# Andreas-Edling/raytracer-rs

Measured on AMD Instinct MI355X. Metric: Mrays/s (whole node) + ms/frame, 1920x1080x64spp thai2.dae, higher is better.
Workload: dtype f32

## Files before the change

### raytracer-rs_amd/csrc/kernels.hip

```cpp
#include <hip/hip_runtime.h>
#include <algorithm>
#include <stdint.h>
#include <stdlib.h>
#include <map>
#include <mutex>
#include <utility>
#include "device_math.hpp"
#include "device_types.hpp"
#include "kernels.hpp"
#include "lens.hpp"
#include "reflmask.hpp"
#include "traverse.hpp"

namespace mi355rt {

typedef const uint32_t __attribute__((address_space(4))) * const_u1_ptr;
constexpr int kBlock = 256;
constexpr int kWavesPerBlock = kBlock / 64;
constexpr uint32_t kMiss = 0xFFFFFFFFu;
constexpr int kPrimaryBlocks = 7;
#ifndef MI355RT_WIDE_BLOCKS
#define MI355RT_WIDE_BLOCKS 5
#endif
constexpr int kConfirmBlocks = 5;
// ... 842 lines not shown
                        float4 tv0 = table[jx0], tv1 = table[jx1];
                        hemisphere_walk(table, n, jx0, tv0);
                        if (two) hemisphere_walk(table, n, jx1, tv1);
                        bd0 = mk3(tv0.x, tv0.y, tv0.z); bo0 = add3(hp, sscale(0.00001f, bd0));
                        bd1 = mk3(tv1.x, tv1.y, tv1.z); bo1 = add3(hp, sscale(0.00001f, bd1));
                    }
                    bool make0 = active, make1 = active && two;
                    if (sc.refl_mask != nullptr) {
                        if (make0) make0 = !reflection_proves_miss(sc, refl_rec, n, bo0, bd0);
                        if (make1) make1 = !reflection_proves_miss(sc, refl_rec, n, bo1, bd1);
                        bskipped += (uint32_t)__popcll(__ballot(active && !make0)) + (uint32_t)__popcll(__ballot(active && two && !make1));
                    }
                    uint32_t pos[2] = { 0u, 0u };
                    const uint32_t key0 = make0 ? dir_bin(bd0) : kSortBins, key1 = make1 ? dir_bin(bd1) : kSortBins;
                    for (uint32_t b = 0; b < kSortBins; ++b) {
                        const unsigned long long m0 = __ballot(key0 == b), m1 = __ballot(key1 == b);
                        if (key0 == b) pos[0] = out_front + (uint32_t)__popcll(m0 & lanemask_lt());
                        out_front += (uint32_t)__popcll(m0);
                        if (key1 == b) pos[1] = out_front + (uint32_t)__popcll(m1 & lanemask_lt());
                        out_front += (uint32_t)__popcll(m1);
                    }
                    for (uint32_t w = 0; w < (two ? 2u : 1u); ++w) {
                        const f3 bo = w ? bo1 : bo0, bd = w ? bd1 : bd0;
                        const uint32_t child_node = w ? child1 : child0;
                        const uint32_t oi = pos[w];
                        if ((w ? make1 : make0) && oi + out_back < ps.region + 0u) {
                            const size_t r = base + oi;
                            st4<2>(&out_q[r], make_float4(bo.x, bo.y, bo.z, bd.x));
                            st4<2>(&out_q[ps.qstride + r], make_float4(bd.y, bd.z, __uint_as_float(slot), __uint_as_float(((level + 1u) << 4) | (child_node << 8))));
                        }
                    }
                }
            }
        }
        __builtin_amdgcn_wave_barrier();
        if (out_front + out_back > ps.region) { if (lane == 0) counters->overflow = 1u; out_front = 0u; out_back = 0u; }
        if (out_counts != nullptr && lane == 0) out_counts[chunk] = make_uint2(out_front, out_back);
        out_nrad = out_front; out_nshadow = out_back;
        acc_bounce += out_front + ((unsigned long long)bskipped << 32); acc_shadow += out_back + ((unsigned long long)skipped << 32); acc_hits += cnt - dropped;
    }
}

__device__ __forceinline__ void flush_shade_counters(DCounters* counters, uint32_t wave, unsigned long long acc_bounce, unsigned long long acc_shadow, unsigned long long acc_hits)
{
    if (lane_id() == 0) {
        DCounters* cs = &counters[wave % kShards];
        if (acc_bounce & 0xFFFFFFFFull) atomicAdd(&cs->bounce, acc_bounce & 0xFFFFFFFFull);
        if (acc_bounce >> 32) atomicAdd(&cs->bounce_skipped, acc_bounce >> 32);
        if (acc_shadow & 0xFFFFFFFFull) atomicAdd(&cs->shadow, acc_shadow & 0xFFFFFFFFull);
        if (acc_shadow >> 32) atomicAdd(&cs->shadow_skipped, acc_shadow >> 32);
        if (acc_hits & 0xFFFFFFFFull) atomicAdd(&cs->primary_hits, acc_hits & 0xFFFFFFFFull);
        if (acc_hits >> 32) atomicAdd(&cs->primary_culled, acc_hits >> 32);
    }
}

template <bool PRIMARY, bool WALK, bool RASTER = false, uint32_t RAYS = kFeedCamera>
__global__ __launch_bounds__(kBlock, PRIMARY ? (WALK ? kShadePWBlocks : kShadePBlocks) : (WALK ? kShadeSWBlocks : kShadeSBlocks)) void shade_kernel(DScene sc, DCamera cam, DPass ps, uint32_t level,
                                                      const float4* __restrict__ in_q, const uint2* __restrict__ in_counts,
                                                      const float4* __restrict__ hits,
                                                      float4* __restrict__ out_q, uint2* __restrict__ out_counts, uint32_t* cursor,
                                                      float* __restrict__ slot_L, uint32_t* __restrict__ sample_slot,
                                                      const uint32_t* __restrict__ film_n, DCounters* counters)
{
    extern __shared__ uint32_t s_list[];
    const LinearList list{ &s_list[(threadIdx.x >> 6) * ps.list_cap] };
    float4* lds_hits = RASTER ? (float4*)&s_list[kWavesPerBlock * ps.list_cap] + (threadIdx.x >> 6) * ps.chunk : nullptr;
    const uint32_t wave = blockIdx.x * kWavesPerBlock + (threadIdx.x >> 6);
    unsigned long long acc_bounce = 0, acc_shadow = 0, acc_hits = 0, acc_tris = 0;
    PullState pull; uint32_t chunk = 0u;
    while (pull_chunk(cursor, ps.nchunks, pull, chunk, 0u, PRIMARY ? LiveLists() : live_lists(ps))) {
        uint32_t o_rad, o_sh;
        shade_chunk<PRIMARY, LinearList, WALK, RASTER, RAYS>(sc, cam, ps, level, chunk, list, in_q, PRIMARY ? 0u : in_counts[chunk].x, o_rad, o_sh, hits, out_q, out_counts, slot_L, sample_slot, film_n, counters, acc_bounce, acc_shadow, acc_hits,
                                                       lds_hits, (RASTER && (ps.flags & 2u)) ? &acc_tris : nullptr);
        if (PRIMARY && ps.live != nullptr && (o_rad | o_sh) != 0u && lane_id() == 0) {
            const uint32_t k = chunk % kMaxCursors;
            const uint32_t at = atomicAdd(&ps.live_count[(size_t)k * kCursorStride + kLiveCountOffset], 1u);
            ps.live[(size_t)k * ps.live_cap + at] = chunk;
        }
    }
    flush_shade_counters(counters, wave, acc_bounce, acc_shadow, PRIMARY ? acc_hits : 0ull);
    if (RASTER && acc_tris && lane_id() == 0) atomicAdd(&counters[wave % kShards].tris_tested, acc_tris);
}

template <int REC>
__device__ f3 node_radiance(const float* __restrict__ L, const DPass& ps, uint32_t nlights, uint32_t level, uint32_t index)
{
    const uint32_t node = ps.level_first[level] + index;
    f3 rad = mk3(0.0f, 0.0f, 0.0f);
    for (uint32_t li = 0; li < nlights; ++li) {
        const float* p = L + 3ull * ((size_t)node * nlights + li) * ps.nslots;
        rad = add3(rad, mk3(p[0], p[1], p[2]));
    }
    if constexpr (REC == 0) {
        return rad;
    } else {
        const uint32_t k = ps.spread * (uint32_t)REC;
        f3 sum = mk3(0.0f, 0.0f, 0.0f);
        for (uint32_t c = 0; c < k; ++c) sum = add3(sum, node_radiance<REC - 1>(L, ps, nlights, level + 1, index * k + c));
        const f3 sub = vscale(sum, div_rn(1.0f, (float)k));
        return add3(rad, sub);
    }
}

template <uint32_t kResolveLanes, bool DIRECT>
__global__ __launch_bounds__(256) void resolve_kernel(DPass ps, uint32_t width, uint32_t nlights, const float* __restrict__ slot_L,
                                                     const uint32_t* __restrict__ sample_slot,
                                                     float* film_sum, float* film_sumsq, uint32_t* film_n, float* debug_color, uint32_t* ctrl, float* film_direct)
{
    if (ctrl != nullptr && blockIdx.x == 0)
        for (uint32_t i = threadIdx.x; i < kMaxRounds * kMaxCursors * 4u; i += blockDim.x)
            ctrl[(size_t)(i / (kMaxCursors * 4u)) * kCtrlWordsPerRound + (size_t)((i / 4u) % kMaxCursors) * kCursorStride + (i % 4u) * kConfirmCursorOffset] = 0u;
    const uint32_t gid = blockIdx.x * blockDim.x + threadIdx.x;
    const uint32_t j = gid % kResolveLanes;
    const bool live = gid / kResolveLanes < ps.npix;
    const uint32_t p = live ? gid / kResolveLanes : ps.npix - 1u;
    const uint32_t spp = ps.nsamples / ps.npix;
    const uint32_t pixel = ps.use_explicit ? ps.explicit_pixel : pass_pixel(ps, width, p);
    f3 sum = mk3(0, 0, 0), sumsq = mk3(0, 0, 0), direct = mk3(0, 0, 0);
    uint32_t n = 0;
    if (!ps.use_explicit) {
        sum = mk3(film_sum[3ull * pixel], film_sum[3ull * pixel + 1], film_sum[3ull * pixel + 2]);
        sumsq = mk3(film_sumsq[3ull * pixel], film_sumsq[3ull * pixel + 1], film_sumsq[3ull * pixel + 2]);
        n = film_n[pixel];
        if constexpr (DIRECT) direct = mk3(film_direct[3ull * pixel], film_direct[3ull * pixel + 1], film_direct[3ull * pixel + 2]);
    }
    const int group_lane0 = lane_id() & ~(int)(kResolveLanes - 1u);
    const bool dead = ps.block_culled != nullptr && ps.block_culled[(uint32_t)(sample_index(ps, 0u, p) / ps.chunk) % ps.cull_blocks] != 0u;
    const bool on = ps.use_explicit || pixel_active(ps, width, pixel);
    for (uint32_t s0 = 0; s0 < spp; s0 += kResolveLanes) {
        const uint32_t sl = (s0 + j < spp && !dead && on) ? sample_slot[sample_index(ps, s0 + j, p)] : 0xFFFFFFFFu;
        const float* L = slot_L + 3ull * (size_t)sl;
        f3 c = mk3(0.0f, 0.0f, 0.0f);
        if (sl != 0xFFFFFFFFu) switch (ps.recursions) {
            case 0: c = node_radiance<0>(L, ps, nlights, 0, 0); break;
            case 1: c = node_radiance<1>(L, ps, nlights, 0, 0); break;
            case 2: c = node_radiance<2>(L, ps, nlights, 0, 0); break;
            default: c = node_radiance<3>(L, ps, nlights, 0, 0); break;
        }
        f3 d = mk3(0.0f, 0.0f, 0.0f);
        if constexpr (DIRECT) { if (sl != 0xFFFFFFFFu) d = node_radiance<0>(L, ps, nlights, 0, 0); }
#pragma unroll
        for (uint32_t k = 0; k < kResolveLanes; ++k) {
            const f3 ck = mk3(__shfl(c.x, group_lane0 + (int)k, 64), __shfl(c.y, group_lane0 + (int)k, 64), __shfl(c.z, group_lane0 + (int)k, 64));
            f3 dk = mk3(0.0f, 0.0f, 0.0f);
            if constexpr (DIRECT) dk = mk3(__shfl(d.x, group_lane0 + (int)k, 64), __shfl(d.y, group_lane0 + (int)k, 64), __shfl(d.z, group_lane0 + (int)k, 64));
            if (s0 + k < spp) {
                sum = add3(sum, ck);
                sumsq = add3(sumsq, mk3(ck.x * ck.x, ck.y * ck.y, ck.z * ck.z));
                n += 1u;
                if constexpr (DIRECT) direct = add3(direct, dk);
                if (ps.use_explicit && j == 0u) { debug_color[0] = ck.x; debug_color[1] = ck.y; debug_color[2] = ck.z; }
            }
        }
    }
    if (!ps.use_explicit && live && on && j == 0u) {
        film_sum[3ull * pixel] = sum.x; film_sum[3ull * pixel + 1] = sum.y; film_sum[3ull * pixel + 2] = sum.z;
        film_sumsq[3ull * pixel] = sumsq.x; film_sumsq[3ull * pixel + 1] = sumsq.y; film_sumsq[3ull * pixel + 2] = sumsq.z;
        film_n[pixel] = n;
        if constexpr (DIRECT) { film_direct[3ull * pixel] = direct.x; film_direct[3ull * pixel + 1] = direct.y; film_direct[3ull * pixel + 2] = direct.z; }
    }
}

__global__ __launch_bounds__(256) void resolve_rays_kernel(DPass ps, uint32_t nlights, const float* __restrict__ slot_L, const uint32_t* __restrict__ sample_slot,
                                                          float* __restrict__ rgb, float* __restrict__ direct, float* __restrict__ tuv, uint32_t* __restrict__ prim, uint32_t* ctrl)
{
    if (ctrl != nullptr && blockIdx.x == 0)
        for (uint32_t i = threadIdx.x; i < kMaxRounds * kMaxCursors * 4u; i += blockDim.x)
            ctrl[(size_t)(i / (kMaxCursors * 4u)) * kCtrlWordsPerRound + (size_t)((i / 4u) % kMaxCursors) * kCursorStride + (i % 4u) * kConfirmCursorOffset] = 0u;
    const uint32_t i = blockIdx.x * blockDim.x + threadIdx.x;
    if (i >= ps.nsamples) return;
    if (rgb != nullptr || direct != nullptr) {
        const uint32_t sl = sample_slot[i];
        const float* L = slot_L + 3ull * (size_t)sl;
        f3 c = mk3(0.0f, 0.0f, 0.0f), d = mk3(0.0f, 0.0f, 0.0f);
        if (sl != 0xFFFFFFFFu) {
            if (rgb != nullptr) switch (ps.recursions) {
                case 0: c = node_radiance<0>(L, ps, nlights, 0, 0); break;
                case 1: c = node_radiance<1>(L, ps, nlights, 0, 0); break;
                case 2: c = node_radiance<2>(L, ps, nlights, 0, 0); break;
                default: c = node_radiance<3>(L, ps, nlights, 0, 0); break;
            }
            if (direct != nullptr) d = node_radiance<0>(L, ps, nlights, 0, 0);
        }
        if (rgb != nullptr) { rgb[3ull * i] = c.x; rgb[3ull * i + 1] = c.y; rgb[3ull * i + 2] = c.z; }
        if (direct != nullptr) { direct[3ull * i] = d.x; direct[3ull * i + 1] = d.y; direct[3ull * i + 2] = d.z; }
    }
    if (ps.ray_hit != nullptr) {
        const float4 h = ps.ray_hit[i];
        const uint32_t p = __float_as_uint(h.w);
        if (prim != nullptr) prim[i] = p;
        if (tuv != nullptr && p != kMiss) { tuv[3ull * i] = h.x; tuv[3ull * i + 1] = h.y; tuv[3ull * i + 2] = h.z; }
    }
}
hipError_t launch_resolve_rays(hipStream_t stream, const DPass& ps, uint32_t nlights, const float* slot_L, const uint32_t* sample_slot,
                               float* rgb, float* direct, float* tuv, uint32_t* prim, uint32_t* ctrl)
{
    hipLaunchKernelGGL(resolve_rays_kernel, dim3((ps.nsamples + 255u) / 256u ? (ps.nsamples + 255u) / 256u : 1u), dim3(256), 0, stream, ps, nlights, slot_L, sample_slot, rgb, direct, tuv, prim, ctrl);
    return hipGetLastError();
}

__device__ __forceinline__ void phase_fence() { __builtin_amdgcn_fence(__ATOMIC_SEQ_CST, "workgroup"); }

template <bool DIRECT>
__device__ __forceinline__ void resolve_chunk_1spp(const DPass& ps, uint32_t width, uint32_t nlights, uint32_t chunk, const float* slot_L, const uint32_t* sample_slot,
                                                   float* film_sum, float* film_sumsq, uint32_t* film_n, float* film_direct)
{
    const uint32_t n = min(ps.chunk, ps.nsamples - chunk * ps.chunk);
    for (uint32_t i = (uint32_t)lane_id(); i < n; i += 64u) {
        const uint32_t p = chunk * ps.chunk + i;
        const uint32_t pixel = pass_pixel(ps, width, p);
        const uint32_t sl = sample_slot[p];
        const float* L = slot_L + 3ull * (size_t)sl;
        f3 c = mk3(0.0f, 0.0f, 0.0f);
        if (sl != 0xFFFFFFFFu) switch (ps.recursions) {
            case 0: c = node_radiance<0>(L, ps, nlights, 0, 0); break;
            case 1: c = node_radiance<1>(L, ps, nlights, 0, 0); break;
            case 2: c = node_radiance<2>(L, ps, nlights, 0, 0); break;
            default: c = node_radiance<3>(L, ps, nlights, 0, 0); break;
        }
        float* ps_ = film_sum + 3ull * pixel; float* pq = film_sumsq + 3ull * pixel;
        ps_[0] = ps_[0] + c.x; ps_[1] = ps_[1] + c.y; ps_[2] = ps_[2] + c.z;
        pq[0] = pq[0] + c.x * c.x; pq[1] = pq[1] + c.y * c.y; pq[2] = pq[2] + c.z * c.z;
        film_n[pixel] = film_n[pixel] + 1u;
        if constexpr (DIRECT) {
            f3 d = mk3(0.0f, 0.0f, 0.0f);
            if (sl != 0xFFFFFFFFu) d = node_radiance<0>(L, ps, nlights, 0, 0);
            float* pd = film_direct + 3ull * pixel;
            pd[0] = pd[0] + d.x; pd[1] = pd[1] + d.y; pd[2] = pd[2] + d.z;
        }
    }
}

constexpr int kFusedBlocks = 1;
template <bool CONFIRM, bool DIRECT>
__global__ __launch_bounds__(kBlock, kFusedBlocks) void fused_pass_kernel(DScene sc, DCamera cam, DPass ps, float4* q0, float4* q1,
                                                            float4* hits, float* slot_L, uint32_t* sample_slot,
                                                            float* film_sum, float* film_sumsq, uint32_t* film_n, float* film_direct, DCounters* counters)
{
    extern __shared__ int s_stack[];
    int* stack = &s_stack[threadIdx.x];
    const ColumnList list{ &s_stack[threadIdx.x & ~63u] };
    const uint32_t wave = global_wave_id(), nwaves = gridDim.x * kWavesPerBlock;
    unsigned long long acc_bounce = 0, acc_shadow = 0, acc_hits = 0;
    for (uint32_t chunk = wave; chunk < ps.nchunks; chunk += nwaves) {
        uint32_t n_rad = 0u, n_sh = 0u;
        trace_wave<true, false, true, true>(sc, cam, ps, nullptr, nullptr, hits, nullptr, slot_L, film_n, counters, stack, chunk, 0u, 0u);
        phase_fence();
        if (CONFIRM && !sc.oct_single_leaf) { confirm_chunk<true>(sc, cam, ps, chunk, list, nullptr, 0u, 0u, hits, slot_L, film_n); phase_fence(); }
        shade_chunk<true>(sc, cam, ps, 0u, chunk, list, nullptr, 0u, n_rad, n_sh, hits, q0, nullptr, slot_L, sample_slot, film_n, counters, acc_bounce, acc_shadow, acc_hits);
        phase_fence();
        for (uint32_t r = 1; r < ps.recursions + 2u; ++r) {
            float4* in_q = (r - 1u) & 1u ? q1 : q0;
            trace_wave<false, false, true, CONFIRM>(sc, cam, ps, in_q, nullptr, hits, nullptr, slot_L, film_n, counters, stack, chunk, n_rad, n_sh);
            phase_fence();
            if (CONFIRM && !sc.oct_single_leaf) { confirm_chunk<false>(sc, cam, ps, chunk, list, in_q, n_rad, n_sh, hits, slot_L, film_n); phase_fence(); }
            if (r <= ps.recursions) {
                unsigned long long unused = 0;
                uint32_t o_rad = 0u, o_sh = 0u;
                shade_chunk<false>(sc, cam, ps, r, chunk, list, in_q, n_rad, o_rad, o_sh, hits, r & 1u ? q1 : q0, nullptr, slot_L, sample_slot, film_n, counters, acc_bounce, acc_shadow, unused);
                n_rad = o_rad; n_sh = o_sh;
                phase_fence();
            }
        }
        resolve_chunk_1spp<DIRECT>(ps, cam.width, sc.nlights, chunk, slot_L, sample_slot, film_sum, film_sumsq, film_n, film_direct);
    }
    flush_shade_counters(counters, wave, acc_bounce, acc_shadow, acc_hits);
}

__device__ __forceinline__ uint32_t to_u8(float c)
{
    const float m = fmaxf(fminf(c, 1.0f), 0.0f) * 255.0f;
    return (uint32_t)m & 0xFFu;
}
__global__ __launch_bounds__(256) void tonemap_kernel(const uint32_t* __restrict__ rows, uint32_t row_base, uint32_t nrows, uint32_t width, int packed,
                                                     const float* __restrict__ film_sum, const uint32_t* __restrict__ film_n, uint32_t* out)
{
    const size_t i = (size_t)blockIdx.x * blockDim.x + threadIdx.x;
    if (i >= (size_t)nrows * width) return;
    const uint32_t r = (uint32_t)(i / width), x = (uint32_t)(i % width);
    const size_t pixel = (size_t)(rows ? rows[r] : row_base + r) * width + x;
    const float inv = div_rn(1.0f, (float)film_n[pixel]);
    const float cr = film_sum[3 * pixel] * inv, cg = film_sum[3 * pixel + 1] * inv, cb = film_sum[3 * pixel + 2] * inv;
    const uint32_t R = to_u8(div_rn(cr, 1.0f + cr)), G = to_u8(div_rn(cg, 1.0f + cg)), B = to_u8(div_rn(cb, 1.0f + cb));
    out[packed ? i : pixel] = B | (G << 8) | (R << 16) | (255u << 24);
}

__device__ __forceinline__ void closest_hit(const DScene& sc, const f3 o, const f3 d, int mode, int* stack, float& t, float& u, float& v, uint32_t& prim)
{
    if (mode == 1) { octree_intersect(sc, o, d, t, u, v, prim); return; }
    RayState rs;
    uint32_t a = 0, b = 0;
    ray_init(rs, o, d, false, sc.root);
    ray_run<false>(sc, rs, stack, kBlock, a, b);
    t = rs.t; u = rs.u; v = rs.v; prim = rs.prim;
    if (mode == 0 && prim != kMiss) confirm_walk(sc, o, d, t, u, v, prim);
}
__global__ __launch_bounds__(kBlock) void intersect_kernel(DScene sc, const float* __restrict__ rays6, uint32_t n, int shadow_mode, int mode,
                                                          float* tuv, uint32_t* prim, uint8_t* blocked)
{
    extern __shared__ int s_stack[];
    const uint32_t i = blockIdx.x * blockDim.x + threadIdx.x;
    if (i >= n) return;
    const f3 o = mk3(rays6[6ull * i], rays6[6ull * i + 1], rays6[6ull * i + 2]);
    const f3 d = mk3(rays6[6ull * i + 3], rays6[6ull * i + 4], rays6[6ull * i + 5]);
    if (!shadow_mode) {
        float t, u, v; uint32_t p;
        closest_hit(sc, o, d, mode, &s_stack[threadIdx.x], t, u, v, p);
        prim[i] = p;
        if (p != kMiss) { tuv[3ull * i] = t; tuv[3ull * i + 1] = u; tuv[3ull * i + 2] = v; }
        return;
    }
// ... 450 lines not shown
    if (rays == kFeedLensOrtho) return count ? launch_trace_variant<true, true, true, kFeedLensOrtho>(MI355RT_TRACE_ARGS) : launch_trace_variant<true, false, true, kFeedLensOrtho>(MI355RT_TRACE_ARGS);
    if (rays) return count ? launch_trace_variant<true, true, true, kFeedRays>(MI355RT_TRACE_ARGS) : launch_trace_variant<true, false, true, kFeedRays>(MI355RT_TRACE_ARGS);
    if (primary) return count ? launch_trace_variant<true, true, true>(MI355RT_TRACE_ARGS) : launch_trace_variant<true, false, true>(MI355RT_TRACE_ARGS);
    if (confirm) return count ? launch_trace_variant<false, true, true>(MI355RT_TRACE_ARGS) : launch_trace_variant<false, false, true>(MI355RT_TRACE_ARGS);
    return count ? launch_trace_variant<false, true, false>(MI355RT_TRACE_ARGS) : launch_trace_variant<false, false, false>(MI355RT_TRACE_ARGS);
#undef MI355RT_TRACE_ARGS
}

__global__ __launch_bounds__(kBlock) void cull_blocks_kernel(DCamera cam, DPass ps, uint32_t nblocks, uint32_t* out)
{
    const uint32_t nwaves = gridDim.x * kWavesPerBlock;
    for (uint32_t b = global_wave_id(); b < nblocks; b += nwaves) {
        const bool culled = chunk_is_culled(cam, ps, b, ps.chunk);
        if (lane_id() == 0) out[b] = culled ? 1u : 0u;
    }
}
hipError_t launch_cull_blocks(hipStream_t stream, const DCamera& cam, const DPass& ps, uint32_t nblocks, uint32_t* out)
{
    if (nblocks == 0) return hipSuccess;
    DPass plain = ps; plain.block_culled = nullptr; plain.cull_blocks = 0;
    const unsigned blocks = std::min<unsigned>((nblocks + kWavesPerBlock - 1) / kWavesPerBlock, 4096u);
    hipLaunchKernelGGL(cull_blocks_kernel, dim3(blocks), dim3(kBlock), 0, stream, cam, plain, nblocks, out);
    return hipGetLastError();
}

hipError_t launch_trace_octree(hipStream_t stream, int num_cus, bool primary, const DScene& sc, const DCamera& cam, const DPass& ps,
                               const void* in_q, const void* in_counts, void* hits, float* slot_L, const uint32_t* film_n, uint32_t rays)
{
    if ((rays && !primary) || rays > kFeedLensOrthoMasked) return hipErrorInvalidValue;
    unsigned blocks = (ps.nchunks + kWavesPerBlock - 1) / kWavesPerBlock;
    const unsigned cap = (unsigned)num_cus * 4u;
    if (blocks > cap) blocks = cap;
    if (blocks < 1) blocks = 1;
    dim3 grid(blocks), block(kBlock);
    if (rays == kFeedLensThinMasked) hipLaunchKernelGGL((trace_octree_kernel<true, kFeedLensThinMasked>), grid, block, 0, stream, sc, cam, ps, (const float4*)in_q, (const uint2*)in_counts, (float4*)hits, slot_L, film_n);
    else if (rays == kFeedLensOrthoMasked) hipLaunchKernelGGL((trace_octree_kernel<true, kFeedLensOrthoMasked>), grid, block, 0, stream, sc, cam, ps, (const float4*)in_q, (const uint2*)in_counts, (float4*)hits, slot_L, film_n);
    else if (rays == kFeedLensThin) hipLaunchKernelGGL((trace_octree_kernel<true, kFeedLensThin>), grid, block, 0, stream, sc, cam, ps, (const float4*)in_q, (const uint2*)in_counts, (float4*)hits, slot_L, film_n);
    else if (rays == kFeedLensOrtho) hipLaunchKernelGGL((trace_octree_kernel<true, kFeedLensOrtho>), grid, block, 0, stream, sc, cam, ps, (const float4*)in_q, (const uint2*)in_counts, (float4*)hits, slot_L, film_n);
    else if (rays) hipLaunchKernelGGL((trace_octree_kernel<true, kFeedRays>), grid, block, 0, stream, sc, cam, ps, (const float4*)in_q, (const uint2*)in_counts, (float4*)hits, slot_L, film_n);
    else if (primary) hipLaunchKernelGGL((trace_octree_kernel<true>), grid, block, 0, stream, sc, cam, ps, (const float4*)in_q, (const uint2*)in_counts, (float4*)hits, slot_L, film_n);
    else hipLaunchKernelGGL((trace_octree_kernel<false>), grid, block, 0, stream, sc, cam, ps, (const float4*)in_q, (const uint2*)in_counts, (float4*)hits, slot_L, film_n);
    return hipGetLastError();
}

hipError_t launch_shade(hipStream_t stream, int num_cus, bool primary, bool walk, const DScene& sc, const DCamera& cam, const DPass& ps, uint32_t level,
                        const void* in_q, const void* in_counts, const void* hits, void* out_q, void* out_counts, uint32_t* cursor,
                        float* slot_L, uint32_t* sample_slot, const uint32_t* film_n, DCounters* counters, bool raster, uint32_t rays)
{
    if ((rays && (!primary || raster)) || rays > kFeedLensOrthoMasked) return hipErrorInvalidValue;
    const size_t lds = (size_t)ps.list_cap * kWavesPerBlock * sizeof(uint32_t) + (raster ? (size_t)ps.chunk * kWavesPerBlock * sizeof(float4) : 0);
    unsigned blocks = (ps.nchunks + kWavesPerBlock - 1) / kWavesPerBlock;
    const unsigned cap = (unsigned)num_cus * (primary ? (walk ? kShadePWBlocks : kShadePBlocks) : (walk ? kShadeSWBlocks : kShadeSBlocks));
    if (blocks > cap) blocks = cap;
    if (blocks < 1) blocks = 1;
    dim3 grid(blocks), block(kBlock);
#define MI355RT_SHADE_ARGS grid, block, lds, stream, sc, cam, ps, level, (const float4*)in_q, (const uint2*)in_counts, (const float4*)hits, (float4*)out_q, (uint2*)out_counts, cursor, slot_L, sample_slot, film_n, counters
    if (rays == kFeedLensThinMasked && walk) hipLaunchKernelGGL((shade_kernel<true, true, false, kFeedLensThinMasked>), MI355RT_SHADE_ARGS);
    else if (rays == kFeedLensThinMasked) hipLaunchKernelGGL((shade_kernel<true, false, false, kFeedLensThinMasked>), MI355RT_SHADE_ARGS);
    else if (rays == kFeedLensOrthoMasked && walk) hipLaunchKernelGGL((shade_kernel<true, true, false, kFeedLensOrthoMasked>), MI355RT_SHADE_ARGS);
    else if (rays == kFeedLensOrthoMasked) hipLaunchKernelGGL((shade_kernel<true, false, false, kFeedLensOrthoMasked>), MI355RT_SHADE_ARGS);
    else if (rays == kFeedLensThin && walk) hipLaunchKernelGGL((shade_kernel<true, true, false, kFeedLensThin>), MI355RT_SHADE_ARGS);
    else if (rays == kFeedLensThin) hipLaunchKernelGGL((shade_kernel<true, false, false, kFeedLensThin>), MI355RT_SHADE_ARGS);
    else if (rays == kFeedLensOrtho && walk) hipLaunchKernelGGL((shade_kernel<true, true, false, kFeedLensOrtho>), MI355RT_SHADE_ARGS);
    else if (rays == kFeedLensOrtho) hipLaunchKernelGGL((shade_kernel<true, false, false, kFeedLensOrtho>), MI355RT_SHADE_ARGS);
    else if (rays && walk) hipLaunchKernelGGL((shade_kernel<true, true, false, kFeedRays>), MI355RT_SHADE_ARGS);
    else if (rays) hipLaunchKernelGGL((shade_kernel<true, false, false, kFeedRays>), MI355RT_SHADE_ARGS);
    else if (primary && raster && walk) hipLaunchKernelGGL((shade_kernel<true, true, true>), MI355RT_SHADE_ARGS);
    else if (primary && raster) hipLaunchKernelGGL((shade_kernel<true, false, true>), MI355RT_SHADE_ARGS);
    else if (primary && walk) hipLaunchKernelGGL((shade_kernel<true, true>), MI355RT_SHADE_ARGS);
    else if (primary) hipLaunchKernelGGL((shade_kernel<true, false>), MI355RT_SHADE_ARGS);
    else if (walk) hipLaunchKernelGGL((shade_kernel<false, true>), MI355RT_SHADE_ARGS);
    else hipLaunchKernelGGL((shade_kernel<false, false>), MI355RT_SHADE_ARGS);
#undef MI355RT_SHADE_ARGS
    return hipGetLastError();
}

hipError_t launch_resolve(hipStream_t stream, const DPass& ps, uint32_t width, uint32_t nlights, const float* slot_L, const uint32_t* sample_slot,
                          float* film_sum, float* film_sumsq, uint32_t* film_n, float* film_direct, float* debug_color, uint32_t* ctrl)
{
    const uint32_t spp = ps.npix ? ps.nsamples / ps.npix : 1u;
    const uint32_t lanes = spp <= 32u ? 2u : (spp <= 96u ? 4u : 8u);
    dim3 block(256), grid((unsigned)(((size_t)ps.npix * lanes + 255) / 256));
#define MI355RT_RESOLVE_ARGS grid, block, 0, stream, ps, width, nlights, slot_L, sample_slot, film_sum, film_sumsq, film_n, debug_color, ctrl, film_direct
    if (film_direct != nullptr && !ps.use_explicit) switch (lanes) {
        case 2: hipLaunchKernelGGL((resolve_kernel<2, true>), MI355RT_RESOLVE_ARGS); break;
        case 4: hipLaunchKernelGGL((resolve_kernel<4, true>), MI355RT_RESOLVE_ARGS); break;
        default: hipLaunchKernelGGL((resolve_kernel<8, true>), MI355RT_RESOLVE_ARGS); break;
    }
    else switch (lanes) {
        case 2: hipLaunchKernelGGL((resolve_kernel<2, false>), MI355RT_RESOLVE_ARGS); break;
        case 4: hipLaunchKernelGGL((resolve_kernel<4, false>), MI355RT_RESOLVE_ARGS); break;
        default: hipLaunchKernelGGL((resolve_kernel<8, false>), MI355RT_RESOLVE_ARGS); break;
    }
#undef MI355RT_RESOLVE_ARGS
    return hipGetLastError();
}

hipError_t launch_tonemap(hipStream_t stream, const uint32_t* rows, uint32_t row_base, uint32_t nrows, uint32_t width, bool packed,
                          const float* film_sum, const uint32_t* film_n, uint32_t* out)
{
    const size_t n = (size_t)nrows * width;
    if (n == 0) return hipSuccess;
    dim3 block(256), grid((unsigned)((n + 255) / 256));
    hipLaunchKernelGGL(tonemap_kernel, grid, block, 0, stream, rows, row_base, nrows, width, packed ? 1 : 0, film_sum, film_n, out);
    return hipGetLastError();
}

template <bool DIRECT>
__device__ __forceinline__ void film_clear_rows_body(const uint32_t* __restrict__ rows, uint32_t nrows, uint32_t width, float* film_sum, float* film_sumsq, uint32_t* film_n, float* film_direct)
{
    const size_t i = (size_t)blockIdx.x * blockDim.x + threadIdx.x;
    if (i >= (size_t)nrows * width) return;
    const size_t pixel = (size_t)rows[i / width] * width + i % width;
    film_sum[3 * pixel] = 0.0f; film_sum[3 * pixel + 1] = 0.0f; film_sum[3 * pixel + 2] = 0.0f;
    film_sumsq[3 * pixel] = 0.0f; film_sumsq[3 * pixel + 1] = 0.0f; film_sumsq[3 * pixel + 2] = 0.0f;
    film_n[pixel] = 0u;
    if constexpr (DIRECT) { film_direct[3 * pixel] = 0.0f; film_direct[3 * pixel + 1] = 0.0f; film_direct[3 * pixel + 2] = 0.0f; }
}
__global__ __launch_bounds__(256) void film_clear_rows_kernel(const uint32_t* __restrict__ rows, uint32_t nrows, uint32_t width, float* film_sum, float* film_sumsq, uint32_t* film_n)
{
    film_clear_rows_body<false>(rows, nrows, width, film_sum, film_sumsq, film_n, nullptr);
}
__global__ __launch_bounds__(256) void film_clear_rows_direct_kernel(const uint32_t* __restrict__ rows, uint32_t nrows, uint32_t width, float* film_sum, float* film_sumsq, uint32_t* film_n,
                                                                    float* film_direct)
{
    film_clear_rows_body<true>(rows, nrows, width, film_sum, film_sumsq, film_n, film_direct);
}
template <bool DIRECT>
__device__ __forceinline__ void film_rows_copy_body(const uint32_t* __restrict__ rows, uint32_t first, uint32_t total, uint32_t nown, uint32_t width,
                                                    float* film_sum, float* film_sumsq, uint32_t* film_n, float* film_direct,
                                                    float* bk_sum, float* bk_sumsq, uint32_t* bk_n, float* bk_direct, int restore)
{
    const size_t i = (size_t)blockIdx.x * blockDim.x + threadIdx.x;
    if (i >= (size_t)total * width) return;
    const uint32_t k = (uint32_t)(i / width), x = (uint32_t)(i % width);
    const size_t pixel = (size_t)rows[(first + k) % nown] * width + x;
    if (restore) {
        film_sum[3 * pixel] = bk_sum[3 * i]; film_sum[3 * pixel + 1] = bk_sum[3 * i + 1]; film_sum[3 * pixel + 2] = bk_sum[3 * i + 2];
        film_sumsq[3 * pixel] = bk_sumsq[3 * i]; film_sumsq[3 * pixel + 1] = bk_sumsq[3 * i + 1]; film_sumsq[3 * pixel + 2] = bk_sumsq[3 * i + 2];
        film_n[pixel] = bk_n[i];
        if constexpr (DIRECT) { film_direct[3 * pixel] = bk_direct[3 * i]; film_direct[3 * pixel + 1] = bk_direct[3 * i + 1]; film_direct[3 * pixel + 2] = bk_direct[3 * i + 2]; }
    } else {
        bk_sum[3 * i] = film_sum[3 * pixel]; bk_sum[3 * i + 1] = film_sum[3 * pixel + 1]; bk_sum[3 * i + 2] = film_sum[3 * pixel + 2];
        bk_sumsq[3 * i] = film_sumsq[3 * pixel]; bk_sumsq[3 * i + 1] = film_sumsq[3 * pixel + 1]; bk_sumsq[3 * i + 2] = film_sumsq[3 * pixel + 2];
        bk_n[i] = film_n[pixel];
        if constexpr (DIRECT) { bk_direct[3 * i] = film_direct[3 * pixel]; bk_direct[3 * i + 1] = film_direct[3 * pixel + 1]; bk_direct[3 * i + 2] = film_direct[3 * pixel + 2]; }
    }
}
__global__ __launch_bounds__(256) void film_rows_copy_kernel(const uint32_t* __restrict__ rows, uint32_t first, uint32_t total, uint32_t nown, uint32_t width,
                                                            float* film_sum, float* film_sumsq, uint32_t* film_n, float* bk_sum, float* bk_sumsq, uint32_t* bk_n, int restore)
{
    film_rows_copy_body<false>(rows, first, total, nown, width, film_sum, film_sumsq, film_n, nullptr, bk_sum, bk_sumsq, bk_n, nullptr, restore);
}
__global__ __launch_bounds__(256) void film_rows_copy_direct_kernel(const uint32_t* __restrict__ rows, uint32_t first, uint32_t total, uint32_t nown, uint32_t width,
                                                                   float* film_sum, float* film_sumsq, uint32_t* film_n, float* film_direct,
                                                                   float* bk_sum, float* bk_sumsq, uint32_t* bk_n, float* bk_direct, int restore)
{
    film_rows_copy_body<true>(rows, first, total, nown, width, film_sum, film_sumsq, film_n, film_direct, bk_sum, bk_sumsq, bk_n, bk_direct, restore);
}
hipError_t launch_film_rows_copy(hipStream_t stream, const uint32_t* rows, uint32_t first, uint32_t total, uint32_t nown, uint32_t width,
                                 float* film_sum, float* film_sumsq, uint32_t* film_n, float* film_direct,
                                 float* bk_sum, float* bk_sumsq, uint32_t* bk_n, float* bk_direct, bool restore)
{
    const size_t n = (size_t)total * width;
    if (n == 0) return hipSuccess;
    if ((film_direct == nullptr) != (bk_direct == nullptr)) return hipErrorInvalidValue;
    const dim3 grid((unsigned)((n + 255) / 256));
    if (film_direct) hipLaunchKernelGGL(film_rows_copy_direct_kernel, grid, dim3(256), 0, stream, rows, first, total, nown, width, film_sum, film_sumsq, film_n, film_direct,
                                        bk_sum, bk_sumsq, bk_n, bk_direct, restore ? 1 : 0);
    else hipLaunchKernelGGL(film_rows_copy_kernel, grid, dim3(256), 0, stream, rows, first, total, nown, width, film_sum, film_sumsq, film_n, bk_sum, bk_sumsq, bk_n, restore ? 1 : 0);
    return hipGetLastError();
}

hipError_t launch_film_clear_rows(hipStream_t stream, const uint32_t* rows, uint32_t nrows, uint32_t width, float* film_sum, float* film_sumsq, uint32_t* film_n, float* film_direct)
{
    const size_t n = (size_t)nrows * width;
// ... 176 lines not shown
```

Measured before the change: 21000.

## Batch resolve radiance loads across samples and flatten small light trees

The resolve kernel now processes U samples per lane at once, so loads from independent slots can be in flight together. When the per-sample node tree is small, it loads every node's radiance in one flat, unrolled pass instead of recursing. Pixels that are culled or inactive skip the sample loop entirely. The cost is higher register pressure and more template instantiations. The flat path hard-codes the tree shape for recursions of two or more (spread of two), which looks specific to the expected configuration.

Measured after the change: 21370 (median of 6 runs). 1.02x the previous value.

```diff
diff --git a/raytracer-rs_amd/csrc/kernels.hip b/raytracer-rs_amd/csrc/kernels.hip
--- a/raytracer-rs_amd/csrc/kernels.hip
+++ b/raytracer-rs_amd/csrc/kernels.hip
@@ -948,27 +948,108 @@
     if (RASTER && acc_tris && lane_id() == 0) atomicAdd(&counters[wave % kShards].tris_tested, acc_tris);
 }
 
-template <int REC>
-__device__ f3 node_radiance(const float* __restrict__ L, const DPass& ps, uint32_t nlights, uint32_t level, uint32_t index)
+template <int REC, uint32_t U>
+__device__ __forceinline__ void node_radiance(const float* __restrict__ slot_L, const uint32_t (&sl)[U], const DPass& ps, uint32_t nlights, uint32_t level, uint32_t index, f3 (&out)[U])
 {
     const uint32_t node = ps.level_first[level] + index;
-    f3 rad = mk3(0.0f, 0.0f, 0.0f);
+    f3 rad[U];
+#pragma unroll
+    for (uint32_t u = 0; u < U; ++u) rad[u] = mk3(0.0f, 0.0f, 0.0f);
     for (uint32_t li = 0; li < nlights; ++li) {
-        const float* p = L + 3ull * ((size_t)node * nlights + li) * ps.nslots;
-        rad = add3(rad, mk3(p[0], p[1], p[2]));
+        f3 t[U];
+#pragma unroll
+        for (uint32_t u = 0; u < U; ++u) {
+            t[u] = mk3(0.0f, 0.0f, 0.0f);
+            if (sl[u] != 0xFFFFFFFFu) {
+                const float* p = slot_L + 3ull * ((size_t)(node * nlights + li) * ps.nslots + sl[u]);
+                t[u] = mk3(p[0], p[1], p[2]);
+            }
+        }
+#pragma unroll
+        for (uint32_t u = 0; u < U; ++u) rad[u] = add3(rad[u], t[u]);
     }
     if constexpr (REC == 0) {
-        return rad;
+#pragma unroll
+        for (uint32_t u = 0; u < U; ++u) out[u] = rad[u];
     } else {
         const uint32_t k = ps.spread * (uint32_t)REC;
-        f3 sum = mk3(0.0f, 0.0f, 0.0f);
-        for (uint32_t c = 0; c < k; ++c) sum = add3(sum, node_radiance<REC - 1>(L, ps, nlights, level + 1, index * k + c));
-        const f3 sub = vscale(sum, div_rn(1.0f, (float)k));
-        return add3(rad, sub);
-    }
-}
-
-template <uint32_t kResolveLanes, bool DIRECT>
+        f3 sum[U];
+#pragma unroll
+        for (uint32_t u = 0; u < U; ++u) sum[u] = mk3(0.0f, 0.0f, 0.0f);
+        for (uint32_t c = 0; c < k; ++c) {
+            f3 child[U];
+            node_radiance<REC - 1, U>(slot_L, sl, ps, nlights, level + 1, index * k + c, child);
+#pragma unroll
+            for (uint32_t u = 0; u < U; ++u) sum[u] = add3(sum[u], child[u]);
+        }
+        const float inv = div_rn(1.0f, (float)k);
+#pragma unroll
+        for (uint32_t u = 0; u < U; ++u) out[u] = add3(rad[u], vscale(sum[u], inv));
+    }
+}
+template <uint32_t U>
+__device__ __forceinline__ void tree_radiance(const float* __restrict__ slot_L, const uint32_t (&sl)[U], const DPass& ps, uint32_t nlights, f3 (&c)[U])
+{
+    switch (ps.recursions) {
+        case 0: node_radiance<0, U>(slot_L, sl, ps, nlights, 0, 0, c); break;
+        case 1: node_radiance<1, U>(slot_L, sl, ps, nlights, 0, 0, c); break;
+        case 2: node_radiance<2, U>(slot_L, sl, ps, nlights, 0, 0, c); break;
+        default: node_radiance<3, U>(slot_L, sl, ps, nlights, 0, 0, c); break;
+    }
+}
+constexpr uint32_t kFlatNodes = 5;
+template <uint32_t U>
+__device__ __forceinline__ void flat_radiance(const float* __restrict__ slot_L, const uint32_t (&sl)[U], const DPass& ps, uint32_t nlights, f3 (&c)[U], f3 (&root)[U])
+{
+    f3 rad[kFlatNodes][U];
+#pragma unroll
+    for (uint32_t q = 0; q < kFlatNodes; ++q) {
+#pragma unroll
+        for (uint32_t u = 0; u < U; ++u) rad[q][u] = mk3(0.0f, 0.0f, 0.0f);
+    }
+    for (uint32_t li = 0; li < nlights; ++li) {
+        f3 t[kFlatNodes][U];
+#pragma unroll
+        for (uint32_t q = 0; q < kFlatNodes; ++q) {
+#pragma unroll
+            for (uint32_t u = 0; u < U; ++u) {
+                t[q][u] = mk3(0.0f, 0.0f, 0.0f);
+                if (sl[u] != 0xFFFFFFFFu && q < ps.nodes_per_sample) {
+                    const float* p = slot_L + 3ull * ((size_t)(q * nlights + li) * ps.nslots + sl[u]);
+                    t[q][u] = mk3(p[0], p[1], p[2]);
+                }
+            }
+        }
+#pragma unroll
+        for (uint32_t q = 0; q < kFlatNodes; ++q) {
+#pragma unroll
+            for (uint32_t u = 0; u < U; ++u) rad[q][u] = add3(rad[q][u], t[q][u]);
+        }
+    }
+#pragma unroll
+    for (uint32_t u = 0; u < U; ++u) {
+        root[u] = rad[0][u];
+        if (ps.recursions == 0u) c[u] = rad[0][u];
+        else if (ps.recursions == 1u) {
+            const uint32_t k = ps.spread;
+            f3 sum = mk3(0.0f, 0.0f, 0.0f);
+#pragma unroll
+            for (uint32_t ci = 0; ci + 1u < kFlatNodes; ++ci) if (ci < k) sum = add3(sum, rad[1u + ci][u]);
+            c[u] = add3(rad[0][u], vscale(sum, div_rn(1.0f, (float)k)));
+        } else {
+            f3 sum = mk3(0.0f, 0.0f, 0.0f);
+#pragma unroll
+            for (uint32_t ci = 0; ci < 2u; ++ci) {
+                const f3 below = add3(mk3(0.0f, 0.0f, 0.0f), rad[3u + ci][u]);
+                sum = add3(sum, add3(rad[1u + ci][u], vscale(below, div_rn(1.0f, 1.0f))));
+            }
+            c[u] = add3(rad[0][u], vscale(sum, div_rn(1.0f, 2.0f)));
+        }
+    }
+}
+
+constexpr uint32_t kResolveU = 2;
+template <uint32_t kResolveLanes, uint32_t U, bool DIRECT, bool FLAT>
 __global__ __launch_bounds__(256) void resolve_kernel(DPass ps, uint32_t width, uint32_t nlights, const float* __restrict__ slot_L,
                                                      const uint32_t* __restrict__ sample_slot,
                                                      float* film_sum, float* film_sumsq, uint32_t* film_n, float* debug_color, uint32_t* ctrl, float* film_direct)
@@ -993,29 +1074,39 @@
     const int group_lane0 = lane_id() & ~(int)(kResolveLanes - 1u);
     const bool dead = ps.block_culled != nullptr && ps.block_culled[(uint32_t)(sample_index(ps, 0u, p) / ps.chunk) % ps.cull_blocks] != 0u;
     const bool on = ps.use_explicit || pixel_active(ps, width, pixel);
-    for (uint32_t s0 = 0; s0 < spp; s0 += kResolveLanes) {
-        const uint32_t sl = (s0 + j < spp && !dead && on) ? sample_slot[sample_index(ps, s0 + j, p)] : 0xFFFFFFFFu;
-        const float* L = slot_L + 3ull * (size_t)sl;
-        f3 c = mk3(0.0f, 0.0f, 0.0f);
-        if (sl != 0xFFFFFFFFu) switch (ps.recursions) {
-            case 0: c = node_radiance<0>(L, ps, nlights, 0, 0); break;
-            case 1: c = node_radiance<1>(L, ps, nlights, 0, 0); break;
-            case 2: c = node_radiance<2>(L, ps, nlights, 0, 0); break;
-            default: c = node_radiance<3>(L, ps, nlights, 0, 0); break;
-        }
-        f3 d = mk3(0.0f, 0.0f, 0.0f);
-        if constexpr (DIRECT) { if (sl != 0xFFFFFFFFu) d = node_radiance<0>(L, ps, nlights, 0, 0); }
+    if (!ps.use_explicit && (dead || !on)) {
+        if (spp != 0u) {
+            sum = add3(sum, mk3(0.0f, 0.0f, 0.0f)); sumsq = add3(sumsq, mk3(0.0f, 0.0f, 0.0f));
+            if constexpr (DIRECT) direct = add3(direct, mk3(0.0f, 0.0f, 0.0f));
+        }
+        n += spp;
+    } else for (uint32_t s0 = 0; s0 < spp; s0 += kResolveLanes * U) {
+        uint32_t sl[U];
 #pragma unroll
-        for (uint32_t k = 0; k < kResolveLanes; ++k) {
-            const f3 ck = mk3(__shfl(c.x, group_lane0 + (int)k, 64), __shfl(c.y, group_lane0 + (int)k, 64), __shfl(c.z, group_lane0 + (int)k, 64));
-            f3 dk = mk3(0.0f, 0.0f, 0.0f);
-            if constexpr (DIRECT) dk = mk3(__shfl(d.x, group_lane0 + (int)k, 64), __shfl(d.y, group_lane0 + (int)k, 64), __shfl(d.z, group_lane0 + (int)k, 64));
-            if (s0 + k < spp) {
-                sum = add3(sum, ck);
-                sumsq = add3(sumsq, mk3(ck.x * ck.x, ck.y * ck.y, ck.z * ck.z));
-                n += 1u;
-                if constexpr (DIRECT) direct = add3(direct, dk);
-                if (ps.use_explicit && j == 0u) { debug_color[0] = ck.x; debug_color[1] = ck.y; debug_color[2] = ck.z; }
+        for (uint32_t u = 0; u < U; ++u) {
+            const uint32_t s = s0 + u * kResolveLanes + j;
+            sl[u] = (s < spp && !dead) ? sample_slot[sample_index(ps, s, p)] : 0xFFFFFFFFu;
+        }
+        f3 c[U], d[U];
+        if constexpr (FLAT) flat_radiance<U>(slot_L, sl, ps, nlights, c, d);
+        else {
+            tree_radiance<U>(slot_L, sl, ps, nlights, c);
+            if constexpr (DIRECT) node_radiance<0, U>(slot_L, sl, ps, nlights, 0, 0, d);
+        }
+#pragma unroll
+        for (uint32_t u = 0; u < U; ++u) {
+#pragma unroll
+            for (uint32_t k = 0; k < kResolveLanes; ++k) {
+                const f3 ck = mk3(__shfl(c[u].x, group_lane0 + (int)k, 64), __shfl(c[u].y, group_lane0 + (int)k, 64), __shfl(c[u].z, group_lane0 + (int)k, 64));
+                f3 dk = mk3(0.0f, 0.0f, 0.0f);
+                if constexpr (DIRECT) dk = mk3(__shfl(d[u].x, group_lane0 + (int)k, 64), __shfl(d[u].y, group_lane0 + (int)k, 64), __shfl(d[u].z, group_lane0 + (int)k, 64));
+                if (s0 + u * kResolveLanes + k < spp) {
+                    sum = add3(sum, ck);
+                    sumsq = add3(sumsq, mk3(ck.x * ck.x, ck.y * ck.y, ck.z * ck.z));
+                    n += 1u;
+                    if constexpr (DIRECT) direct = add3(direct, dk);
+                    if (ps.use_explicit && j == 0u) { debug_color[0] = ck.x; debug_color[1] = ck.y; debug_color[2] = ck.z; }
+                }
             }
         }
     }
@@ -1036,20 +1127,12 @@
     const uint32_t i = blockIdx.x * blockDim.x + threadIdx.x;
     if (i >= ps.nsamples) return;
     if (rgb != nullptr || direct != nullptr) {
-        const uint32_t sl = sample_slot[i];
-        const float* L = slot_L + 3ull * (size_t)sl;
-        f3 c = mk3(0.0f, 0.0f, 0.0f), d = mk3(0.0f, 0.0f, 0.0f);
-        if (sl != 0xFFFFFFFFu) {
-            if (rgb != nullptr) switch (ps.recursions) {
-                case 0: c = node_radiance<0>(L, ps, nlights, 0, 0); break;
-                case 1: c = node_radiance<1>(L, ps, nlights, 0, 0); break;
-                case 2: c = node_radiance<2>(L, ps, nlights, 0, 0); break;
-                default: c = node_radiance<3>(L, ps, nlights, 0, 0); break;
-            }
-            if (direct != nullptr) d = node_radiance<0>(L, ps, nlights, 0, 0);
-        }
-        if (rgb != nullptr) { rgb[3ull * i] = c.x; rgb[3ull * i + 1] = c.y; rgb[3ull * i + 2] = c.z; }
-        if (direct != nullptr) { direct[3ull * i] = d.x; direct[3ull * i + 1] = d.y; direct[3ull * i + 2] = d.z; }
+        const uint32_t sl[1] = { sample_slot[i] };
+        f3 c[1] = { mk3(0.0f, 0.0f, 0.0f) }, d[1] = { mk3(0.0f, 0.0f, 0.0f) };
+        if (rgb != nullptr) tree_radiance<1>(slot_L, sl, ps, nlights, c);
+        if (direct != nullptr) node_radiance<0, 1>(slot_L, sl, ps, nlights, 0, 0, d);
+        if (rgb != nullptr) { rgb[3ull * i] = c[0].x; rgb[3ull * i + 1] = c[0].y; rgb[3ull * i + 2] = c[0].z; }
+        if (direct != nullptr) { direct[3ull * i] = d[0].x; direct[3ull * i + 1] = d[0].y; direct[3ull * i + 2] = d[0].z; }
     }
     if (ps.ray_hit != nullptr) {
         const float4 h = ps.ray_hit[i];
@@ -1075,24 +1158,19 @@
     for (uint32_t i = (uint32_t)lane_id(); i < n; i += 64u) {
         const uint32_t p = chunk * ps.chunk + i;
         const uint32_t pixel = pass_pixel(ps, width, p);
-        const uint32_t sl = sample_slot[p];
-        const float* L = slot_L + 3ull * (size_t)sl;
-        f3 c = mk3(0.0f, 0.0f, 0.0f);
-        if (sl != 0xFFFFFFFFu) switch (ps.recursions) {
-            case 0: c = node_radiance<0>(L, ps, nlights, 0, 0); break;
-            case 1: c = node_radiance<1>(L, ps, nlights, 0, 0); break;
-            case 2: c = node_radiance<2>(L, ps, nlights, 0, 0); break;
-            default: c = node_radiance<3>(L, ps, nlights, 0, 0); break;
-        }
+        const uint32_t sl[1] = { sample_slot[p] };
+        f3 c1[1];
+        tree_radiance<1>(slot_L, sl, ps, nlights, c1);
+        const f3 c = c1[0];
         float* ps_ = film_sum + 3ull * pixel; float* pq = film_sumsq + 3ull * pixel;
         ps_[0] = ps_[0] + c.x; ps_[1] = ps_[1] + c.y; ps_[2] = ps_[2] + c.z;
         pq[0] = pq[0] + c.x * c.x; pq[1] = pq[1] + c.y * c.y; pq[2] = pq[2] + c.z * c.z;
         film_n[pixel] = film_n[pixel] + 1u;
         if constexpr (DIRECT) {
-            f3 d = mk3(0.0f, 0.0f, 0.0f);
-            if (sl != 0xFFFFFFFFu) d = node_radiance<0>(L, ps, nlights, 0, 0);
+            f3 d[1];
+            node_radiance<0, 1>(slot_L, sl, ps, nlights, 0, 0, d);
             float* pd = film_direct + 3ull * pixel;
-            pd[0] = pd[0] + d.x; pd[1] = pd[1] + d.y; pd[2] = pd[2] + d.z;
+            pd[0] = pd[0] + d[0].x; pd[1] = pd[1] + d[0].y; pd[2] = pd[2] + d[0].z;
         }
     }
 }
@@ -1709,16 +1787,17 @@
     const uint32_t lanes = spp <= 32u ? 2u : (spp <= 96u ? 4u : 8u);
     dim3 block(256), grid((unsigned)(((size_t)ps.npix * lanes + 255) / 256));
 #define MI355RT_RESOLVE_ARGS grid, block, 0, stream, ps, width, nlights, slot_L, sample_slot, film_sum, film_sumsq, film_n, debug_color, ctrl, film_direct
-    if (film_direct != nullptr && !ps.use_explicit) switch (lanes) {
-        case 2: hipLaunchKernelGGL((resolve_kernel<2, true>), MI355RT_RESOLVE_ARGS); break;
-        case 4: hipLaunchKernelGGL((resolve_kernel<4, true>), MI355RT_RESOLVE_ARGS); break;
-        default: hipLaunchKernelGGL((resolve_kernel<8, true>), MI355RT_RESOLVE_ARGS); break;
-    }
-    else switch (lanes) {
-        case 2: hipLaunchKernelGGL((resolve_kernel<2, false>), MI355RT_RESOLVE_ARGS); break;
-        case 4: hipLaunchKernelGGL((resolve_kernel<4, false>), MI355RT_RESOLVE_ARGS); break;
-        default: hipLaunchKernelGGL((resolve_kernel<8, false>), MI355RT_RESOLVE_ARGS); break;
-    }
+#define MI355RT_RESOLVE_LANES(DIRECT, FLAT) switch (lanes) { \
+        case 2: hipLaunchKernelGGL((resolve_kernel<2, kResolveU, DIRECT, FLAT>), MI355RT_RESOLVE_ARGS); break; \
+        case 4: hipLaunchKernelGGL((resolve_kernel<4, kResolveU, DIRECT, FLAT>), MI355RT_RESOLVE_ARGS); break; \
+        default: hipLaunchKernelGGL((resolve_kernel<8, kResolveU, DIRECT, FLAT>), MI355RT_RESOLVE_ARGS); break; }
+    const bool direct = film_direct != nullptr && !ps.use_explicit;
+    const bool flat = ps.nodes_per_sample <= kFlatNodes;
+    if (direct && flat) MI355RT_RESOLVE_LANES(true, true)
+    else if (direct) MI355RT_RESOLVE_LANES(true, false)
+    else if (flat) MI355RT_RESOLVE_LANES(false, true)
+    else MI355RT_RESOLVE_LANES(false, false)
+#undef MI355RT_RESOLVE_LANES
 #undef MI355RT_RESOLVE_ARGS
     return hipGetLastError();
 }
```
